# forbes110/taiwan-whisper

Hardware: AMD Instinct MI355X
Metric: distillation utterances/sec (30 s clips) (higher is better)
Workload: dtype bf16

## Files before the change

### include/tw_hip.h

```cpp
#ifndef TW_HIP_H
#define TW_HIP_H
#include <stdint.h>
#ifdef __cplusplus
extern "C" {
#endif

typedef void* tw_stream_t;

#define TW_GEMM_BIAS 1
#define TW_GEMM_ROUND 2
#define TW_GEMM_GELU 4
#define TW_GEMM_RES 8
#define TW_GEMM_ACCUM 16
#define TW_GEMM_AUX_OUT 32
#define TW_GEMM_DGELU 64
#define TW_GEMM_TILE128 256
#define TW_GEMM_TILE256 512
#define TW_GEMM_TILE256x128 1024
#define TW_GEMM_TILE256PP 2048
#define TW_GEMM_NOSPLIT 16384
#define TW_GEMM_TILE256x128_S2 262144
#define TW_GEMM_GROUP_M(g) ((g) << 24)


// ... 26 lines not shown
int tw_attn_fwd(const void* Q, int64_t ldq, const void* K, int64_t ldk, const void* V, int64_t ldv, void* O,
                int64_t ldo, float* lse, int B, int H, int Tq, int Tk, int head_dim, int causal, float scale,
                tw_stream_t stream);
int tw_attn_bwd(const void* Q, int64_t ldq, const void* K, int64_t ldk, const void* V, int64_t ldv, const void* O,
                int64_t ldo, const void* dO, int64_t lddo, const float* lse, void* dQ, int64_t lddq, void* dK,
                int64_t lddk, void* dV, int64_t lddv, int B, int H, int Tq, int Tk, int head_dim, int causal,
                float scale, float* workspace , tw_stream_t stream);
int tw_attn_fwd_varlen(const void* Q, int64_t ldq, const void* K, int64_t ldk, const void* V, int64_t ldv, void* O,
                       int64_t ldo, float* lse, const int* offq, const int* offk, int B, int H, int Mq, int max_q, int Tk,
                       int head_dim, int causal, float scale, tw_stream_t stream);
int tw_attn_fwd_varlen_f16(const void* Q, int64_t ldq, const void* K, int64_t ldk, const void* V, int64_t ldv, void* O,
                           int64_t ldo, float* lse, const int* offq, const int* offk, int B, int H, int Mq, int max_q,
                           int Tk, int head_dim, int causal, float scale, tw_stream_t stream);
int tw_attn_bwd_varlen(const void* Q, int64_t ldq, const void* K, int64_t ldk, const void* V, int64_t ldv,
                       const void* O, int64_t ldo, const void* dO, int64_t lddo, const float* lse, void* dQ,
                       int64_t lddq, void* dK, int64_t lddk, void* dV, int64_t lddv, const int* offq, const int* offk,
                       int B, int H, int Mq, int max_q, int Tk, int head_dim, int causal, float scale,
                       float* workspace , tw_stream_t stream);
int tw_attn_bwd_varlen_f16(const void* Q, int64_t ldq, const void* K, int64_t ldk, const void* V, int64_t ldv,
                           const void* O, int64_t ldo, const void* dO, int64_t lddo, const float* lse, void* dQ,
                           int64_t lddq, void* dK, int64_t lddk, void* dV, int64_t lddv, const int* offq,
                           const int* offk, int B, int H, int Mq, int max_q, int Tk, int head_dim, int causal,
                           float scale, float* workspace, tw_stream_t stream);

int tw_kl_ce(const void* s_logits, const void* t_logits, int64_t ld, int logits_dtype, const int64_t* labels,
             int64_t rows, int V, float T, float ce_w, float kl_w, const int* n_valid, float grad_scale, float* row_out,
             float* out3, void* dlogits, tw_stream_t stream);

int tw_logmel(const float* wav, int B, const float* basis, const int* mel_start, const float* mel_w, float* mel_out,
              void* conv_in, void* workspace , tw_stream_t stream);
int tw_logmel_len(const float* wav, int B, int64_t n_samples, const float* basis, const int* mel_start,
                  const float* mel_w, float* mel_out, void* conv_in, void* workspace, tw_stream_t stream);
int tw_logmel_mels(const float* wav, int B, int64_t n_samples, int n_mels, const float* basis, const int* mel_start,
                   const float* mel_w, float* mel_out, void* conv_in, void* workspace, tw_stream_t stream);
int tw_mel_to_conv_input(const float* mel, void* xt, int B, int nmel, int T, tw_stream_t stream);

int tw_embed_fwd(const int64_t* ids, const void* tok, int tok_dtype, const void* pos, int pos_dtype, void* out,
                 int out_dtype, int rows, int T, int pos_offset, int D, tw_stream_t stream);
int tw_embed_bwd(const int64_t* ids, const float* dh, float* dE, int rows, int D, int64_t padding_idx,
                 tw_stream_t stream);
int tw_pack_plan(const int64_t* labels, int B, int T, int* off, int64_t* src_rows, tw_stream_t stream);
int tw_embed_fwd_rows(const int64_t* ids, const int64_t* src_rows, const void* tok, int tok_dtype, const void* pos,
                      int pos_dtype, void* out, int out_dtype, int rows, int T, int pos_offset, int D,
                      tw_stream_t stream);
int tw_pos_grad_rows(const float* dx, const int* off, int B, int max_rows, int D, float* gP, tw_stream_t stream);

int tw_transpose_bf16(const void* src, int64_t ld_src, int rows, int cols, void* dst, int64_t ld_dst,
                      tw_stream_t stream);
int tw_cast_f32_bf16(const float* src, void* dst, int64_t n, tw_stream_t stream);
int tw_colsum(const void* x, int x_dtype, int64_t ldx, int rows, int cols, float* out, int accum, int round_bf16,
              float* workspace, int64_t workspace_floats, tw_stream_t stream);

int tw_l2norm(const float* x, int64_t n, float* norm_out, float* workspace , tw_stream_t stream);
int tw_adamw(float* p, const float* g, float* m, float* v, void* p_bf16, int64_t n, float lr, float b1, float b2,
             float eps, float wd, int step, const float* norm, float max_norm, tw_stream_t stream);
int tw_clip_scale(float* x, int64_t n, const float* norm, float max_norm, tw_stream_t stream);

int tw_im2col3(const void* src, int64_t src_rows, void* dst, int B, int T_out, int stride, int C,
               tw_stream_t stream);
int tw_col2im_s2(const float* dA, float* dX, int B, int T_in, int T_out, int C, tw_stream_t stream);
int tw_gelu_bwd(const void* g, int g_dtype, const void* pre, void* out, int64_t n, tw_stream_t stream);

int tw_shift_tokens_right(const int64_t* labels, int64_t* out, int B, int T, int64_t pad, int64_t start,
                          tw_stream_t stream);
// ... 116 lines not shown
```

### taiwan-whisper_amd/csrc/attention.hip

```cpp
#include "common.h"

#include <cstdlib>
#include <type_traits>

namespace {

constexpr int QW = 32;
constexpr int QB = 4 * QW;
constexpr int KT = 64;
constexpr int TB = KT * 64 * 2;

typedef __attribute__((address_space(3))) s16x4 lds_s16x4;

__device__ __forceinline__ int swz(int r, int c) { return r * 128 + ((c ^ (r & 7)) << 4); }

__device__ __forceinline__ void stage_tile(const bf16* base, int64_t ld, int rows_valid, char* lds, int wave,
                                           int lane) {
  const auto rs = make_rsrc(base);
#pragma unroll
  for (int i = 0; i < 2; ++i) {
    const int pce = wave + 4 * i;
    const int r = pce * 8 + (lane >> 3);
    const int c = (lane & 7) ^ (r & 7);
    const uint32_t off = r < rows_valid ? (uint32_t)(((int64_t)r * ld + c * 8) * 2) : TW_OOB;
// ... 32 lines not shown
}

template <bool H>
__device__ __forceinline__ void store4(bf16* dst, const f32x4& v) {
  *(bf16x4*)dst = bf16x4{f2e<H>(v[0]), f2e<H>(v[1]), f2e<H>(v[2]), f2e<H>(v[3])};
}

template <int N, int M>
__device__ __forceinline__ void zero(f32x4 (&a)[N][M]) {
#pragma unroll
  for (int i = 0; i < N; ++i)
#pragma unroll
    for (int j = 0; j < M; ++j) a[i][j] = f32x4{0.f, 0.f, 0.f, 0.f};
}

struct AttnP {
  const bf16* Q; const bf16* K; const bf16* V; bf16* O; float* lse;
  const bf16* dO; float* Dv; bf16* dQ; bf16* dK; bf16* dV;
  int64_t ldq, ldk, ldv, ldo, lddo, lddq, lddk, lddv;
  int B, H, Tq, Tk, causal;
  float scale, scale_log2;
  const int* offq; const int* offk;
  int Mq;
};

template <bool VL>
__device__ __forceinline__ void clip_rows(const int* off, int b, int& T, int64_t& row0) {
  row0 = (int64_t)b * T;
  if constexpr (VL) {
    if (off) {
      row0 = off[b];
      T = off[b + 1] - off[b];
    }
  }
}

constexpr float LOG2E = 1.4426950408889634f;

__device__ __forceinline__ void remap_bh(int& xblk, int& bh) {
  const int nx = gridDim.x, nwg = gridDim.x * gridDim.y;
  const int bid = blockIdx.y * nx + blockIdx.x;
  const int q = nwg / 8, rr = nwg % 8, xcd = bid % 8;
  const int tid = (xcd < rr ? xcd * (q + 1) : rr * (q + 1) + (xcd - rr) * q) + bid / 8;
  bh = tid / nx;
  xblk = tid % nx;
}
constexpr float NEG_BIG = -1e30f;

__device__ __forceinline__ float fmx(float a, float b) { return __builtin_elementwise_maximum(a, b); }

struct Frame {
  int lane, wave, g, li;
  int h;
  int blk, row;
  int Tq, Tk;
  int off;
  int64_t qrow0, krow0;
  int64_t lse0;
  const bf16 *Qb, *Kb, *Vb;
  template <class T> __device__ __forceinline__ T* qrow(T* base, int64_t ld, int r = 0) const {
    return base + (qrow0 + r) * ld + h * 64;
  }
  template <class T> __device__ __forceinline__ T* krow(T* base, int64_t ld, int r = 0) const {
    return base + (krow0 + r) * ld + h * 64;
  }
};

template <bool VL>
__device__ __forceinline__ Frame attn_frame(const AttnP& p) {
  Frame f;
  f.lane = lane_id();
  f.wave = wave_id_uniform();
  f.g = f.lane >> 4;
  f.li = f.lane & 15;
  int xblk, bh;
  remap_bh(xblk, bh);
  const int b = bh / p.H;
  f.h = bh % p.H;
  f.blk = xblk * QB;
  f.row = f.blk + f.wave * QW;
  f.Tq = p.Tq;
  f.Tk = p.Tk;
  clip_rows<VL>(p.offq, b, f.Tq, f.qrow0);
  clip_rows<VL>(p.offk, b, f.Tk, f.krow0);
  f.lse0 = VL ? (int64_t)f.h * p.Mq + f.qrow0 : (int64_t)bh * f.Tq;
  f.Qb = f.qrow(p.Q, p.ldq);
  f.Kb = f.krow(p.K, p.ldk);
  f.Vb = f.krow(p.V, p.ldv);
  f.off = f.Tk - f.Tq;
  return f;
}

__device__ __forceinline__ void stage_kv(const AttnP& p, const Frame& f, char* smem, int buf, int kt) {
  char* Ks = smem + buf * 2 * TB;
  const int k0 = kt * KT;
  stage_tile(f.Kb + (int64_t)k0 * p.ldk, p.ldk, f.Tk - k0, Ks, f.wave, f.lane);
  stage_tile(f.Vb + (int64_t)k0 * p.ldv, p.ldv, f.Tk - k0, Ks + TB, f.wave, f.lane);
}

__device__ __forceinline__ int causal_nkt(const AttnP& p, const Frame& f) {
  int nkt = (f.Tk + KT - 1) / KT;
  if (p.causal) {
// ... 374 lines not shown
    if (!(p.offq != nullptr && p.B > 0 && p.Mq >= 0 && p.Tq >= 0 && p.Tq <= p.Mq && p.Tk >= 0 &&
          !(p.causal && p.Tq > p.Tk)))
      return TW_EINVAL;
    if (p.Tk == 0 || (!bwd && (p.Mq == 0 || p.Tq == 0))) return TW_OK;
  } else if (p.B <= 0 || p.Tq <= 0 || p.Tk <= 0) {
    return TW_OK;
  }
  if ((((uintptr_t)p.Q | (uintptr_t)p.K | (uintptr_t)p.V) & 15) || ((p.ldq | p.ldk | p.ldv) & 7)) return TW_EINVAL;
  if (bwd ? (((uintptr_t)p.dO | (uintptr_t)p.O) & 15) || ((p.lddo | p.ldo) & 7) : (p.ldo & 3) != 0) return TW_EINVAL;
  if (!packed && p.causal && p.Tq > p.Tk) return TW_EINVAL;
  return ATTN_LAUNCH;
}

#define TW_DISPATCH_HVL(half, packed, ...)                                      \
  do {                                                                          \
    if ((half) && (packed)) { constexpr bool H = true, VL = true; __VA_ARGS__; } \
    else if (half) { constexpr bool H = true, VL = false; __VA_ARGS__; }        \
    else if (packed) { constexpr bool H = false, VL = true; __VA_ARGS__; }      \
    else { constexpr bool H = false, VL = false; __VA_ARGS__; }                 \
  } while (0)

dim3 attn_grid(const AttnP& p, int rows) { return dim3((rows + QB - 1) / QB, p.B * p.H); }

int attn_fwd(const AttnP& p, int head_dim, bool packed, bool half, hipStream_t stream) {
  if (const int st = attn_check(p, head_dim, packed, false); st != ATTN_LAUNCH) return st;
  TW_DISPATCH_HVL(half, packed,
                  hipLaunchKernelGGL((attn_fwd_kernel<H, VL>), attn_grid(p, p.Tq), dim3(256), 0, stream, p));
  TW_CHECK_LAUNCH();
  return TW_OK;
}

int attn_bwd(const AttnP& p, int head_dim, bool packed, bool half, hipStream_t stream) {
  if (const int st = attn_check(p, head_dim, packed, true); st != ATTN_LAUNCH) return st;
  TW_DISPATCH_HVL(half, packed, {
    if (p.Tq > 0)
      hipLaunchKernelGGL((attn_bwd_dq_kernel<H, VL>), attn_grid(p, p.Tq), dim3(256), 0, stream, p);
    hipLaunchKernelGGL((attn_bwd_dkdv_kernel<H, VL>), attn_grid(p, p.Tk), dim3(256), 0, stream, p);
  });
  TW_CHECK_LAUNCH();
  return TW_OK;
}

}

extern "C" int tw_attn_fwd(const void* Q, int64_t ldq, const void* K, int64_t ldk, const void* V, int64_t ldv, void* O,
                           int64_t ldo, float* lse, int B, int H, int Tq, int Tk, int head_dim, int causal, float scale,
                           hipStream_t stream) {
  return attn_fwd(attn_fill(Q, ldq, K, ldk, V, ldv, O, ldo, lse, B, H, Tq, Tk, causal, scale, nullptr, nullptr, 0),
                  head_dim, false, false, stream);
}

extern "C" int tw_attn_fwd_f16(const void* Q, int64_t ldq, const void* K, int64_t ldk, const void* V, int64_t ldv,
                               void* O, int64_t ldo, float* lse, int B, int H, int Tq, int Tk, int head_dim, int causal,
                               float scale, hipStream_t stream) {
  return attn_fwd(attn_fill(Q, ldq, K, ldk, V, ldv, O, ldo, lse, B, H, Tq, Tk, causal, scale, nullptr, nullptr, 0),
                  head_dim, false, true, stream);
}

extern "C" int tw_attn_bwd(const void* Q, int64_t ldq, const void* K, int64_t ldk, const void* V, int64_t ldv,
// ... 30 lines not shown
                  head_dim, true, true, stream);
}

extern "C" int tw_attn_bwd_varlen(const void* Q, int64_t ldq, const void* K, int64_t ldk, const void* V, int64_t ldv,
                                  const void* O, int64_t ldo, const void* dO, int64_t lddo, const float* lse, void* dQ,
                                  int64_t lddq, void* dK, int64_t lddk, void* dV, int64_t lddv, const int* offq,
                                  const int* offk, int B, int H, int Mq, int max_q, int Tk, int head_dim, int causal,
                                  float scale, float* workspace, hipStream_t stream) {
  return attn_bwd(attn_fill(Q, ldq, K, ldk, V, ldv, O, ldo, lse, B, H, max_q, Tk, causal, scale, offq, offk, Mq, dO,
                            lddo, dQ, lddq, dK, lddk, dV, lddv, workspace),
                  head_dim, true, false, stream);
}

extern "C" int tw_attn_bwd_varlen_f16(const void* Q, int64_t ldq, const void* K, int64_t ldk, const void* V,
                                      int64_t ldv, const void* O, int64_t ldo, const void* dO, int64_t lddo,
                                      const float* lse, void* dQ, int64_t lddq, void* dK, int64_t lddk, void* dV,
                                      int64_t lddv, const int* offq, const int* offk, int B, int H, int Mq, int max_q,
                                      int Tk, int head_dim, int causal, float scale, float* workspace,
                                      hipStream_t stream) {
  return attn_bwd(attn_fill(Q, ldq, K, ldk, V, ldv, O, ldo, lse, B, H, max_q, Tk, causal, scale, offq, offk, Mq, dO,
                            lddo, dQ, lddq, dK, lddk, dV, lddv, workspace),
                  head_dim, true, true, stream);
}
```

### taiwan-whisper_amd/csrc/misc.hip

```cpp
#include "common.h"

namespace {

__global__ void embed_fwd_kernel(const int64_t* __restrict__ ids, const void* __restrict__ tok, int tok_dtype,
                                 const void* __restrict__ pos, int pos_dtype, void* __restrict__ out, int out_dtype,
                                 int rows, int T, int pos_offset, int D) {
  const int row = blockIdx.x;
  if (row >= rows) return;
  const int64_t id = ids[row];
  const int t = row % T + pos_offset;
  for (int e = threadIdx.x; e < D; e += blockDim.x) {
    const float a = ld_as_f32(tok, tok_dtype, id * D + e);
    const float b = ld_as_f32(pos, pos_dtype, (int64_t)t * D + e);
    const float s = a + b;
    st_from_f32(out, out_dtype, (int64_t)row * D + e, s);
  }
}

__global__ __launch_bounds__(1024) void pack_plan_kernel(const int64_t* __restrict__ labels, int B, int T, int* off,
                                                         int64_t* __restrict__ src) {
  const int lane = threadIdx.x & 63, wv = threadIdx.x >> 6;
  for (int b = wv; b < B; b += 16) {
    int n = 0;
    for (int t = lane; t < T; t += 64)
      if (labels[(int64_t)b * T + t] >= 0) n = t + 1;
    for (int o = 32; o > 0; o >>= 1) n = max(n, __shfl_xor(n, o, 64));
    if (lane == 0) off[b + 1] = n;
  }
  __syncthreads();
  if (threadIdx.x == 0) {
    int s = 0;
    off[0] = 0;
    for (int b = 0; b < B; ++b) {
      s += off[b + 1];
      off[b + 1] = s;
    }
  }
  __syncthreads();
  for (int b = wv; b < B; b += 16) {
    const int r0 = off[b], n = off[b + 1] - r0;
    for (int t = lane; t < n; t += 64) src[r0 + t] = (int64_t)b * T + t;
  }
  for (int64_t i = off[B] + threadIdx.x; i < (int64_t)B * T; i += 1024) src[i] = 0;
}

__global__ void embed_fwd_rows_kernel(const int64_t* __restrict__ ids, const int64_t* __restrict__ src,
                                      const void* __restrict__ tok, int tok_dtype, const void* __restrict__ pos,
                                      int pos_dtype, void* __restrict__ out, int out_dtype, int rows, int T,
                                      int pos_offset, int D) {
  const int row = blockIdx.x;
  if (row >= rows) return;
  const int64_t id = ids[row];
  const int t = (int)(src[row] % T) + pos_offset;
  for (int e = threadIdx.x; e < D; e += blockDim.x) {
    const float a = ld_as_f32(tok, tok_dtype, id * D + e);
    const float b = ld_as_f32(pos, pos_dtype, (int64_t)t * D + e);
    st_from_f32(out, out_dtype, (int64_t)row * D + e, a + b);
  }
}

__global__ __launch_bounds__(256) void pos_grad_rows_kernel(const float* __restrict__ dx, const int* __restrict__ off,
                                                            int B, int D, float* __restrict__ gP) {
  const int t = blockIdx.x;
  const int e = blockIdx.y * 256 + threadIdx.x;
  if (e >= D) return;
  float acc = 0.f;
// ... 204 lines not shown
  if (b > cap) b = cap;
  if (b < 1) b = 1;
  return (int)b;
}

}

extern "C" int tw_embed_fwd(const int64_t* ids, const void* tok, int tok_dtype, const void* pos, int pos_dtype,
                            void* out, int out_dtype, int rows, int T, int pos_offset, int D, hipStream_t stream) {
  if (rows <= 0) return TW_OK;
  hipLaunchKernelGGL(embed_fwd_kernel, dim3(rows), dim3(256), 0, stream, ids, tok, tok_dtype, pos, pos_dtype, out,
                     out_dtype, rows, T, pos_offset, D);
  TW_CHECK_LAUNCH();
  return TW_OK;
}

extern "C" int tw_pack_plan(const int64_t* labels, int B, int T, int* off, int64_t* src_rows, hipStream_t stream) {
  if (B <= 0 || T <= 0) return TW_EINVAL;
  hipLaunchKernelGGL(pack_plan_kernel, dim3(1), dim3(1024), 0, stream, labels, B, T, off, src_rows);
  TW_CHECK_LAUNCH();
  return TW_OK;
}

extern "C" int tw_embed_fwd_rows(const int64_t* ids, const int64_t* src_rows, const void* tok, int tok_dtype,
                                 const void* pos, int pos_dtype, void* out, int out_dtype, int rows, int T,
                                 int pos_offset, int D, hipStream_t stream) {
  if (rows <= 0) return TW_OK;
  if (T <= 0) return TW_EINVAL;
  hipLaunchKernelGGL(embed_fwd_rows_kernel, dim3(rows), dim3(256), 0, stream, ids, src_rows, tok, tok_dtype, pos,
                     pos_dtype, out, out_dtype, rows, T, pos_offset, D);
  TW_CHECK_LAUNCH();
  return TW_OK;
}

extern "C" int tw_pos_grad_rows(const float* dx, const int* off, int B, int max_rows, int D, float* gP,
                                hipStream_t stream) {
  if (B <= 0 || max_rows <= 0 || D <= 0) return TW_OK;
  hipLaunchKernelGGL(pos_grad_rows_kernel, dim3(max_rows, (D + 255) / 256), dim3(256), 0, stream, dx, off, B, D, gP);
  TW_CHECK_LAUNCH();
  return TW_OK;
}

namespace {

__global__ __launch_bounds__(256) void transpose_bf16_kernel(const bf16* __restrict__ src, int64_t lds_, int rows,
                                                             int cols, bf16* __restrict__ dst, int64_t ldd, int vec) {
// ... 172 lines not shown
```

### taiwan-whisper_amd/tw/_native.py

```python
from __future__ import annotations

import ctypes
import os

_HERE = os.path.dirname(os.path.abspath(__file__))
LIB_PATH = os.environ.get("TW_HIP_LIB", os.path.join(_HERE, "_lib", "libtw_hip.so"))

P, I64, I32, F32 = ctypes.c_void_p, ctypes.c_int64, ctypes.c_int, ctypes.c_float

SIGNATURES = {
    "tw_gemm_bf16": [P, I64, I32, P, I64, I32, P, I64, I32, I32, I32, I32, I32, I64, I64, I64, F32, P,
                     P, I64, I64, I32, I32, P, I64, I64, I32, P],
    "tw_gemm_route": [P, I64, I32, P, I64, I32, P, I64, I32, I32, I32, I32, I32, I64, I64, I64, P,
                      P, I64, I64, I32, I32, P, I64, I64, I32, I32, I32, I32, P],
    "tw_flac_info": [P, I64, P],
    "tw_flac_decode": [P, I64, P, I64, P],
    "tw_gemv_bf16": [P, I64, P, P, F32, P, I64, P, I64, I32, I32, I32, I32, P, P, I64, I32, P, I64, I32,
                     P, I64, I64, I32, P, P],
    "tw_layernorm_fwd": [P, I32, P, P, P, I32, P, P, I32, I32, F32, P],
    "tw_layernorm_bwd": [P, I32, P, P, P, P, I32, P, I32, P, P, I32, I32, P, I64, P],
    "tw_layernorm_bwd_ex": [P, I32, P, P, P, P, I32, P, I32, P, P, I32, I32, P, I64, P, I32, P],
    "tw_add_layernorm_fwd": [P, I32, P, P, P, P, P, P, P, I32, I32, F32, P],
    "tw_attn_fwd": [P, I64, P, I64, P, I64, P, I64, P, I32, I32, I32, I32, I32, I32, F32, P],
    "tw_attn_bwd": [P, I64, P, I64, P, I64, P, I64, P, I64, P, P, I64, P, I64, P, I64, I32, I32, I32, I32,
                    I32, I32, F32, P, P],
    "tw_attn_fwd_varlen": [P, I64, P, I64, P, I64, P, I64, P, P, P, I32, I32, I32, I32, I32, I32, I32, F32, P],
    "tw_attn_fwd_varlen_f16": [P, I64, P, I64, P, I64, P, I64, P, P, P, I32, I32, I32, I32, I32, I32, I32, F32, P],
    "tw_attn_bwd_varlen": [P, I64, P, I64, P, I64, P, I64, P, I64, P, P, I64, P, I64, P, I64, P, P, I32, I32, I32,
                           I32, I32, I32, I32, F32, P, P],
    "tw_attn_bwd_varlen_f16": [P, I64, P, I64, P, I64, P, I64, P, I64, P, P, I64, P, I64, P, I64, P, P, I32, I32,
                               I32, I32, I32, I32, I32, F32, P, P],
    "tw_pack_plan": [P, I32, I32, P, P, P],
    "tw_embed_fwd_rows": [P, P, P, I32, P, I32, P, I32, I32, I32, I32, I32, P],
    "tw_pos_grad_rows": [P, P, I32, I32, I32, P, P],
    "tw_kl_ce": [P, P, I64, I32, P, I64, I32, F32, F32, F32, P, F32, P, P, P, P],
    "tw_logmel": [P, I32, P, P, P, P, P, P, P],
    "tw_logmel_len": [P, I32, I64, P, P, P, P, P, P, P],
    "tw_logmel_mels": [P, I32, I64, I32, P, P, P, P, P, P, P],
    "tw_mel_to_conv_input": [P, P, I32, I32, I32, P],
    "tw_embed_fwd": [P, P, I32, P, I32, P, I32, I32, I32, I32, I32, P],
    "tw_embed_bwd": [P, P, P, I32, I32, I64, P],
    "tw_cast_f32_bf16": [P, P, I64, P],
    "tw_transpose_bf16": [P, I64, I32, I32, P, I64, P],
    "tw_colsum": [P, I32, I64, I32, I32, P, I32, I32, P, I64, P],
    "tw_l2norm": [P, I64, P, P, P],
    "tw_adamw": [P, P, P, P, P, I64, F32, F32, F32, F32, F32, I32, P, F32, P],
    "tw_clip_scale": [P, I64, P, F32, P],
    "tw_im2col3": [P, I64, P, I32, I32, I32, I32, P],
    "tw_col2im_s2": [P, P, I32, I32, I32, I32, P],
    "tw_gelu_bwd": [P, I32, P, P, I64, P],
    "tw_shift_tokens_right": [P, P, I32, I32, I64, I64, P],
    "tw_count_valid": [P, I64, P, P],
    "tw_decode_attn": [P, I64, P, I64, I64, P, I64, I64, P, I64, I32, I32, I32, P, I32, F32, I32, P],
    "tw_decode_attn_hs": [P, I64, P, I64, I64, I64, P, I64, I64, I64, P, I64, I32, I32, I32, P, I32, F32, I32, P],
    "tw_decode_attn_ks": [P, I64, P, I64, I64, I64, P, I64, I64, I64, P, I64, I32, I32, I32, P, P, I32, F32, I32, P],
# ... 69 lines not shown
```

### taiwan-whisper_amd/tw/distill.py

```python
from __future__ import annotations

import contextlib
import math
import os
from typing import Optional

import torch

from . import ops as F
from .modeling import Backward, PackedRows, WhisperForConditionalGeneration, is_pseudo


def constant_with_warmup(step: int, warmup: int) -> float:
    if warmup > 0 and step < warmup:
        return step / warmup
    return 1.0


def linear_schedule(step: int, warmup: int, total: int) -> float:
    if warmup > 0 and step < warmup:
        return step / warmup
    return max(0.0, (total - step) / max(1, total - warmup))


# ... 126 lines not shown
        if self.sched == "constant":
            return self.lr
        return self.lr * constant_with_warmup(step, self.warmup)

    def _conv_input(self, batch):
        ci = batch.get("conv_input")
        if ci is not None and ci.dtype == self.s.act_dtype:
            return ci
        return self.s.conv_input(batch["input_features"])

    def _teacher_logits(self, conv_in, ids, labels, enc16, Tk, pk=None):
        t = self.t
        if self.share:
            t_ids = torch.empty_like(labels)
            F.shift_tokens_right(labels, t_ids, t.config.pad_token_id, t.config.decoder_start_token_id)
            ht = t.decode(t_ids if pk is None else pk.pack(t_ids), enc16, Tk, pk=pk)
        else:
            enc_t = t.encode(conv_in)
            ht = t.decode(ids if pk is None else pk.pack(ids), enc_t, Tk, pk=pk)
        return t.lm_head(ht)

    def _plan_rows(self, batch_labels, labels):
        B, T = labels.shape
        off = torch.empty(B + 1, dtype=torch.int32, device=labels.device)
        src = torch.empty(B * T, dtype=torch.int64, device=labels.device)
        F.pack_plan(labels, off, src)
        def descriptor(lens):
            pk = PackedRows(lens, off, src, T)
            return pk if pk.M > 0 else None

        if not batch_labels.is_cuda:
            pos = torch.arange(1, T + 1, dtype=torch.int64)
            lens = ((batch_labels >= 0) * pos).amax(1).tolist()
            return lambda: descriptor(lens)
        host = self._pin.get(B)
        if host is None:
            host = self._pin[B] = torch.empty(B + 1, dtype=torch.int32).pin_memory()
        host.copy_(off, non_blocking=True)
        ev = torch.cuda.Event()
        ev.record()

        def done():
            ev.synchronize()
            o = host.tolist()
            return descriptor([o[b + 1] - o[b] for b in range(B)])
        return done

    def train_step(self, batch, temperature: Optional[float] = None, end_of_dataloader: bool = False):
        T = self.temperature if temperature is None else temperature
        s = self.s
        conv_in = self._conv_input(batch)
        ids = batch["decoder_input_ids"].to(s.device).contiguous()
        labels = batch["labels"].to(s.device).contiguous()
        B, Td = ids.shape
        plan = self._plan_rows(batch["labels"], labels) if self.pack_rows else None
        enc_tape = [] if self.train_encoder else None
        enc16 = s.encode(conv_in, tape=enc_tape)
        self.flush()
        pk = plan() if plan is not None else None
        if self.micro == 0:
            s.grad.zero_()
        self._pending, self._reduced = [], []
        sync = self.micro + 1 == self.accum or end_of_dataloader
        self.bw.on_ready = self._grad_ready if (self.dp and sync) else None
        Tk = enc16.shape[0] // B
        tape = []
        with self._row_capacity(pk, B * Td):
            hs = s.decode(ids if pk is None else pk.pack(ids), enc16, Tk, tape=tape, pk=pk)
# ... 242 lines not shown
```

### taiwan-whisper_amd/tw/modeling.py

```python
from __future__ import annotations

import json
import math
import os
from dataclasses import dataclass
from typing import Optional

import numpy as np
import torch

from . import ops
from .config import GenerationConfig, WhisperConfig

_DEFER_RES = os.environ.get("TW_DEFER_RES", "1")
_LN_G16 = os.environ.get("TW_LN_G16", "1") != "0"

F = ops


def padded_vocab(V: int) -> int:
    return (V + 63) // 64 * 64



class PackedRows:

    def __init__(self, lens, off, src, T):
        self.lens = [int(n) for n in lens]
        self.B, self.T = len(self.lens), int(T)
        self.M, self.max_len = sum(self.lens), max(self.lens, default=0)
        if self.max_len > self.T or min(self.lens, default=0) < 0:
            raise ValueError("packed rows: a clip length outside [0, T]")
        if off.dtype != torch.int32 or off.numel() < self.B + 1 or src.dtype != torch.int64 or src.numel() < self.M:
            raise ValueError("packed rows: off is int32 [B+1], src int64 [>= M]")
        self.off, self.src = off, src[: self.M]

    @classmethod
    def from_lens(cls, lens, T, device):
        lens = [int(n) for n in lens]
        off = torch.tensor(np.concatenate([[0], np.cumsum(lens)]), dtype=torch.int32, device=device)
        src = torch.tensor([b * T + t for b, n in enumerate(lens) for t in range(n)], dtype=torch.int64, device=device)
        return cls(lens, off, src, T)

    def pack(self, x):
        if tuple(x.shape) != (self.B, self.T):
            raise ValueError(f"packed rows: expected [{self.B}, {self.T}], got {tuple(x.shape)}")
        return x.reshape(-1).index_select(0, self.src)


def fp32_compute_supported() -> bool:
    return True

def _attn_segs(p, d, fused_kv_only=False):
    segs = []
    if not fused_kv_only:
        segs += [(p + ".q_proj.weight", (d, d)), (p + ".k_proj.weight", (d, d)), (p + ".v_proj.weight", (d, d)),
                 (p + ".q_proj.bias", (d,)), (p + ".k_proj.zero_bias", (d,)), (p + ".v_proj.bias", (d,))]
    else:
# ... 420 lines not shown
        return xn, y

    def _res_out(self, h, w, b, x, tape, kind, clamp=False):
        M, N = h.shape[0], w.shape[0]
        if self.defer_residual(kind):
            r = self._rows(M, N, self.act_dtype)
            self._lin(h, w, b, r)
            return x, r
        out = self._rows(M, N, self.stream_dtype) if tape is not None else x
        flags = F.GEMM_ROUND | (F.GEMM_CLAMP16 if clamp and self.stream_dtype == torch.float16 else 0)
        self._lin(h, w, b, out, res=x, flags=flags)
        return out, None

    def _attn_fwd(self, x, p, q, ldq, k, v, ldkv, B, T, Tk, causal, tape, pk):
        d = self.config.d_model
        H = d // 64
        M = B * T if pk is None else pk.M
        o = self._rows(M, d, self.act_dtype)
        lse = torch.empty(H * M, dtype=torch.float32, device=self.device) if tape is not None else None
        if pk is None:
            F.attn_fwd(q, ldq, k, ldkv, v, ldkv, o, d, lse, B, H, T, T if Tk is None else Tk, causal, 0.125)
        else:
            offk, Tk = (pk.off, pk.max_len) if Tk is None else (None, Tk)
            F.attn_fwd_varlen(q, ldq, k, ldkv, v, ldkv, o, d, lse, pk.off, offk, pk.B, H, M, pk.max_len, Tk, causal, 0.125)
        out = self._res_out(o, self._w16(p + ".out_proj.weight"), self._w16(p + ".out_proj.bias"), x, tape, "attn")
        return out, o, lse

    def _attn_block(self, x, p, B, T, causal, tape=None, pend=None, pk=None):
        d = self.config.d_model
        sv = {} if tape is not None else None
        x, y = self._ln_in(x, pend, p + "_layer_norm", sv)
        M = B * T if pk is None else pk.M
        qkv = self._rows(M, 3 * d, self.act_dtype)
        wqkv = self.wspan(p + ".q_proj.weight", p + ".v_proj.weight", (3 * d, d))
        bqkv = self.wspan(p + ".q_proj.bias", p + ".v_proj.bias", (3 * d,))
        self._lin(y, wqkv, bqkv, qkv)
        out, o, lse = self._attn_fwd(x, p, qkv, 3 * d, qkv[:, d:], qkv[:, 2 * d:], 3 * d, B, T, None, causal, tape, pk)
        if tape is not None:
            tape.append(("attn", p, dict(sv=sv, y=y, qkv=qkv, o=o, lse=lse, B=B, T=T, causal=causal, pk=pk)))
        return out

    def _cross_block(self, x, enc16, p, B, T, Tk, tape=None, kv=None, pend=None, pk=None):
        d = self.config.d_model
        sv = {} if tape is not None else None
        x, y = self._ln_in(x, pend, p + "_layer_norm", sv)
        M = B * T if pk is None else pk.M
        q = self._rows(M, d, self.act_dtype)
# ... 260 lines not shown

    def _out_proj(self, p, st, dx):
        m = self.m
        d = m.config.d_model
        pk = st.get("pk")
        M = st["B"] * st["T"] if pk is None else pk.M
        g = self._grad16(dx)
        self.dW(g, st["o"], m.gv(p + ".out_proj.weight"), M)
        self.db(g, (0, d), m.gv(p + ".out_proj.bias"))
        do = m._rows(M, d, m.act_dtype)
        self.dX(g, m._w16(p + ".out_proj.weight"), do)
        return M, do

    def _attn_bwd(self, st, q, ldq, k, v, ldkv, do, dq, lddq, dk, dv, lddkv, Tk, causal):
        d = self.m.config.d_model
        H = d // 64
        B, T, pk = st["B"], st["T"], st.get("pk")
        if pk is None:
            F.attn_bwd(q, ldq, k, ldkv, v, ldkv, st["o"], d, do, d, st["lse"], dq, lddq, dk, lddkv, dv, lddkv, B, H, T,
                       T if Tk is None else Tk, causal, 0.125)
        else:
            offk, Tk = (pk.off, pk.max_len) if Tk is None else (None, Tk)
            F.attn_bwd_varlen(q, ldq, k, ldkv, v, ldkv, st["o"], d, do, d, st["lse"], dq, lddq, dk, lddkv, dv, lddkv,
                              pk.off, offk, pk.B, H, pk.M, pk.max_len, Tk, causal, 0.125)

    def attn(self, p, st, dx):
        m = self.m
        d = m.config.d_model
        M, do = self._out_proj(p, st, dx)
        qkv = st["qkv"]
        dqkv = m._rows(M, 3 * d, m.act_dtype)
        self._attn_bwd(st, qkv, 3 * d, qkv[:, d:], qkv[:, 2 * d:], 3 * d, do, dqkv, 3 * d, dqkv[:, d:], dqkv[:, 2 * d:],
                       3 * d, None, st["causal"])
        self.dW(dqkv, st["y"], self.span_grad(p + ".q_proj.weight", p + ".v_proj.weight", (3 * d, d)), M)
        self.db(dqkv, (0, d), m.gv(p + ".q_proj.bias"))
        self.db(dqkv, (2 * d, 3 * d), m.gv(p + ".v_proj.bias"))
        dy = m._rows(M, d, m.act_dtype)
        wqkv = m.wspan(p + ".q_proj.weight", p + ".v_proj.weight", (3 * d, d))
        self.dX(dqkv, wqkv, dy)
        self.ln(st["sv"], p + "_layer_norm", dy, dx)

    def cross(self, p, st, dx, enc16, d_enc):
        m = self.m
        d = m.config.d_model
        B, Tk = st["B"], st["Tk"]
        M, do = self._out_proj(p, st, dx)
        kv = st["kv"]
# ... 119 lines not shown
```

### taiwan-whisper_amd/tw/ops.py

```python
from __future__ import annotations

import collections
import ctypes

import torch

from ._native import call
from .profiling import KernelTimer

F32, BF16, F16 = 0, 1, 2
GEMM_BIAS, GEMM_ROUND, GEMM_GELU, GEMM_RES, GEMM_ACCUM, GEMM_AUX_OUT, GEMM_DGELU = 1, 2, 4, 8, 16, 32, 64
GEMM_CLAMP16 = 128
HALF = (torch.bfloat16, torch.float16)
GEMM_TILE128, GEMM_TILE256, GEMM_TILE256x128, GEMM_TILE256PP = 256, 512, 1024, 2048
GEMM_NOSPLIT = 16384
GEMM_TILE256x128_S2 = 262144


def GEMM_GROUP_M(g: int) -> int:
    assert 0 < g < 16
    return g << 24


GEMM_ROUTES = ("skinny", "skinny_splitk", "splitk_dw", "rounds_sk_tail", "rounds_dp_tail", "persistent",
# ... 197 lines not shown
def attn_fwd(q, ldq, k, ldk, v, ldv, o, ldo, lse, B, H, Tq, Tk, causal, scale):
    if q.dtype == torch.float32:
        return attn_fwd_f32(q, ldq, k, ldk, v, ldv, o, ldo, lse, B, H, Tq, Tk, causal, scale)
    sym = _attn_sym("attn_fwd", q, ((q, ldq, "q"), (o, ldo, "o")), ((k, ldk, "k"), (v, ldv, "v")), lse, H, B, Tq, Tk)
    call(sym, q.data_ptr(), ldq, k.data_ptr(), ldk, v.data_ptr(), ldv, o.data_ptr(), ldo, _ptr(lse), B, H, Tq, Tk, 64,
         int(causal), float(scale), _stream())
    return o


def attn_bwd(q, ldq, k, ldk, v, ldv, o, ldo, do, lddo, lse, dq, lddq, dk, lddk, dv, lddv, B, H, Tq, Tk, causal,
             scale, workspace=None):
    if q.dtype == torch.float32:
        return attn_bwd_f32(q, ldq, k, ldk, v, ldv, o, ldo, do, lddo, lse, dq, lddq, dk, lddk, dv, lddv, B, H, Tq, Tk,
                            causal, scale)
    sym = _attn_sym("attn_bwd", q, ((q, ldq, "q"), (o, ldo, "o"), (do, lddo, "do"), (dq, lddq, "dq")),
                    ((k, ldk, "k"), (v, ldv, "v"), (dk, lddk, "dk"), (dv, lddv, "dv")), lse, H, B, Tq, Tk)
    if workspace is None or workspace.numel() < B * H * Tq:
        workspace = torch.empty(B * H * Tq, dtype=torch.float32, device=q.device)
    call(sym, q.data_ptr(), ldq, k.data_ptr(), ldk, v.data_ptr(), ldv, o.data_ptr(), ldo, do.data_ptr(), lddo,
         lse.data_ptr(), dq.data_ptr(), lddq, dk.data_ptr(), lddk, dv.data_ptr(), lddv, B, H, Tq, Tk, 64, int(causal),
         float(scale), workspace.data_ptr(), _stream())


def attn_fwd_varlen(q, ldq, k, ldk, v, ldv, o, ldo, lse, offq, offk, B, H, Mq, max_q, Tk, causal, scale):
    sym = _attn_sym("attn_fwd_varlen", q, ((q, ldq, "q"), (o, ldo, "o")), ((k, ldk, "k"), (v, ldv, "v")), lse, H, B,
                    max_q, Tk, offq, offk, Mq)
    if sym is not None:
        call(sym, q.data_ptr(), ldq, k.data_ptr(), ldk, v.data_ptr(), ldv, o.data_ptr(), ldo, _ptr(lse),
             offq.data_ptr(), _ptr(offk), B, H, Mq, max_q, Tk, 64, int(causal), float(scale), _stream())
    return o


def attn_bwd_varlen(q, ldq, k, ldk, v, ldv, o, ldo, do, lddo, lse, dq, lddq, dk, lddk, dv, lddv, offq, offk, B, H, Mq,
                    max_q, Tk, causal, scale):
    sym = _attn_sym("attn_bwd_varlen", q, ((q, ldq, "q"), (o, ldo, "o"), (do, lddo, "do"), (dq, lddq, "dq")),
                    ((k, ldk, "k"), (v, ldv, "v"), (dk, lddk, "dk"), (dv, lddv, "dv")), lse, H, B, max_q, Tk, offq,
                    offk, Mq)
    if sym is None:
        return
    ws = torch.empty(max(H * Mq, 1), dtype=torch.float32, device=q.device)
    call(sym, q.data_ptr(), ldq, k.data_ptr(), ldk, v.data_ptr(), ldv, o.data_ptr(), ldo, do.data_ptr(), lddo,
         lse.data_ptr(), dq.data_ptr(), lddq, dk.data_ptr(), lddk, dv.data_ptr(), lddv, offq.data_ptr(), _ptr(offk), B,
         H, Mq, max_q, Tk, 64, int(causal), float(scale), ws.data_ptr(), _stream())


def kl_ce(s_logits, t_logits, labels, V, n_valid, T=2.0, ce_w=0.8, kl_w=1.0, grad_scale=1.0, dlogits=None,
          row_out=None, out3=None):
    rows, ld = s_logits.shape
    assert t_logits.shape == s_logits.shape and s_logits.dtype == t_logits.dtype
    assert s_logits.dtype in (torch.bfloat16, torch.float16, torch.float32)
    assert labels.dtype == torch.int64 and labels.numel() == rows and n_valid.dtype == torch.int32
    if row_out is None:
        row_out = torch.empty(rows * 2, dtype=torch.float32, device=s_logits.device)
    if out3 is None:
        out3 = torch.empty(3, dtype=torch.float32, device=s_logits.device)
    if dlogits is not None:
        assert dlogits.shape == s_logits.shape and dlogits.dtype == s_logits.dtype
        assert dlogits.data_ptr() != t_logits.data_ptr(), "kl_ce: dlogits may alias the student logits, not the teacher's"
    call("tw_kl_ce", s_logits.data_ptr(), t_logits.data_ptr(), ld, _dt(s_logits), labels.data_ptr(), rows, V, float(T),
         float(ce_w), float(kl_w), n_valid.data_ptr(), float(grad_scale), row_out.data_ptr(), out3.data_ptr(),
         _ptr(dlogits), _stream())
    return out3, row_out


def logmel(wav, basis, mel_start, mel_w, mel_out, conv_in=None, workspace=None):
    B, n = wav.shape
# ... 27 lines not shown
        return xt
    assert xt.dtype in HALF
    call("tw_mel_to_conv_input_f16" if xt.dtype == torch.float16 else "tw_mel_to_conv_input", mel.data_ptr(),
         xt.data_ptr(), B, nmel, T, _stream())
    return xt


def embed_fwd(ids, tok, pos, out, T, pos_offset=0):
    rows = ids.numel()
    D = tok.shape[1]
    assert ids.dtype == torch.int64 and out.shape[-1] == D and out.numel() == rows * D
    assert pos.shape[0] >= T + pos_offset
    call("tw_embed_fwd", ids.data_ptr(), tok.data_ptr(), _dt(tok), pos.data_ptr(), _dt(pos), out.data_ptr(),
         _dt(out), rows, T, pos_offset, D, _stream())
    return out


def pack_plan(labels, off, src_rows):
    B, T = labels.shape
    assert labels.dtype == torch.int64 and labels.is_contiguous() and labels.is_cuda
    assert off.dtype == torch.int32 and src_rows.dtype == torch.int64
    _need(off, B + 1, "pack_plan off"); _need(src_rows, B * T, "pack_plan src_rows")
    call("tw_pack_plan", labels.data_ptr(), B, T, off.data_ptr(), src_rows.data_ptr(), _stream())


def embed_fwd_rows(ids, src_rows, tok, pos, out, T, pos_offset=0):
    rows = ids.numel()
    D = tok.shape[1]
    assert ids.dtype == torch.int64 and src_rows.dtype == torch.int64 and ids.is_contiguous()
    assert out.shape[-1] == D and out.numel() == rows * D and out.is_contiguous()
    assert pos.shape[0] >= T + pos_offset
    _need(src_rows, rows, "embed src_rows")
    call("tw_embed_fwd_rows", ids.data_ptr(), src_rows.data_ptr(), tok.data_ptr(), _dt(tok), pos.data_ptr(), _dt(pos),
         out.data_ptr(), _dt(out), rows, T, pos_offset, D, _stream())
    return out


def pos_grad_rows(dx, off, B, M, max_rows, gP):
    D = gP.shape[1]
    assert dx.dtype == torch.float32 and gP.dtype == torch.float32 and off.dtype == torch.int32
    assert gP.is_contiguous() and gP.shape[0] >= max_rows and 0 <= max_rows <= M
    _need(off, B + 1, "pos_grad off")
    if M > 0:
        _need(dx, M * D, "pos_grad dx")
    call("tw_pos_grad_rows", dx.data_ptr(), off.data_ptr(), B, max_rows, D, gP.data_ptr(), _stream())

# ... 496 lines not shown
```

Measured before the change: 269.7.

## Launch varlen attention over a compact list of live query blocks

Adds a GPU kernel that builds a compact list of (batch, query-block) entries for packed variable-length decoder sequences. For causal attention the list is sorted by KV tile count, longest first. The varlen attention forward and dQ backward kernels are then launched over this list instead of a max_q-by-B grid, so workgroups that would find no valid rows are never created and heavy blocks start first. It adds a small single-workgroup O(n^2) ranking kernel per step and a custom block-to-head placement, and it depends on block counts matching the host-side lengths.

```diff
diff --git a/include/tw_hip.h b/include/tw_hip.h
--- a/include/tw_hip.h
+++ b/include/tw_hip.h
@@ -72,6 +72,24 @@
                            int64_t lddq, void* dK, int64_t lddk, void* dV, int64_t lddv, const int* offq,
                            const int* offk, int B, int H, int Mq, int max_q, int Tk, int head_dim, int causal,
                            float scale, float* workspace, tw_stream_t stream);
+int tw_attn_fwd_blocks(const void* Q, int64_t ldq, const void* K, int64_t ldk, const void* V, int64_t ldv, void* O,
+                       int64_t ldo, float* lse, const int* offq, const int* offk, const int* blocks, int nblk,
+                       int B, int H, int Mq, int max_q, int Tk, int head_dim, int causal, float scale,
+                       tw_stream_t stream);
+int tw_attn_fwd_blocks_f16(const void* Q, int64_t ldq, const void* K, int64_t ldk, const void* V, int64_t ldv, void* O,
+                           int64_t ldo, float* lse, const int* offq, const int* offk, const int* blocks, int nblk,
+                           int B, int H, int Mq, int max_q, int Tk, int head_dim, int causal, float scale,
+                           tw_stream_t stream);
+int tw_attn_bwd_blocks(const void* Q, int64_t ldq, const void* K, int64_t ldk, const void* V, int64_t ldv,
+                       const void* O, int64_t ldo, const void* dO, int64_t lddo, const float* lse, void* dQ,
+                       int64_t lddq, void* dK, int64_t lddk, void* dV, int64_t lddv, const int* offq, const int* offk,
+                       const int* blocks, int nblk, int B, int H, int Mq, int max_q, int Tk, int head_dim, int causal,
+                       float scale, float* workspace , tw_stream_t stream);
+int tw_attn_bwd_blocks_f16(const void* Q, int64_t ldq, const void* K, int64_t ldk, const void* V, int64_t ldv,
+                           const void* O, int64_t ldo, const void* dO, int64_t lddo, const float* lse, void* dQ,
+                           int64_t lddq, void* dK, int64_t lddk, void* dV, int64_t lddv, const int* offq,
+                           const int* offk, const int* blocks, int nblk, int B, int H, int Mq, int max_q, int Tk,
+                           int head_dim, int causal, float scale, float* workspace, tw_stream_t stream);
 
 int tw_kl_ce(const void* s_logits, const void* t_logits, int64_t ld, int logits_dtype, const int64_t* labels,
              int64_t rows, int V, float T, float ce_w, float kl_w, const int* n_valid, float grad_scale, float* row_out,
@@ -90,6 +108,7 @@
 int tw_embed_bwd(const int64_t* ids, const float* dh, float* dE, int rows, int D, int64_t padding_idx,
                  tw_stream_t stream);
 int tw_pack_plan(const int64_t* labels, int B, int T, int* off, int64_t* src_rows, tw_stream_t stream);
+int tw_pack_blocks(const int* off, int B, int max_rows, int* blocks, int cap, int* nblk, tw_stream_t stream);
 int tw_embed_fwd_rows(const int64_t* ids, const int64_t* src_rows, const void* tok, int tok_dtype, const void* pos,
                       int pos_dtype, void* out, int out_dtype, int rows, int T, int pos_offset, int D,
                       tw_stream_t stream);
diff --git a/taiwan-whisper_amd/csrc/attention.hip b/taiwan-whisper_amd/csrc/attention.hip
--- a/taiwan-whisper_amd/csrc/attention.hip
+++ b/taiwan-whisper_amd/csrc/attention.hip
@@ -78,6 +78,7 @@
   float scale, scale_log2;
   const int* offq; const int* offk;
   int Mq;
+  const int4* wl;
 };
 
 template <bool VL>
@@ -122,6 +123,25 @@
   }
 };
 
+__device__ __forceinline__ void place_entry(bool causal, int& ent, int& h) {
+  if (!causal) {
+    remap_bh(h, ent);
+    return;
+  }
+  const int H = gridDim.x, nent = gridDim.y;
+  const int bid = blockIdx.y * H + blockIdx.x;
+  const int full = nent & ~7;
+  if (bid < full * H) {
+    const int t = bid >> 3;
+    h = t % H;
+    ent = (t / H) * 8 + (bid & 7);
+  } else {
+    const int local = bid - full * H, r = nent - full;
+    ent = full + local % r;
+    h = local / r;
+  }
+}
+
 template <bool VL>
 __device__ __forceinline__ Frame attn_frame(const AttnP& p) {
   Frame f;
@@ -129,11 +149,20 @@
   f.wave = wave_id_uniform();
   f.g = f.lane >> 4;
   f.li = f.lane & 15;
-  int xblk, bh;
-  remap_bh(xblk, bh);
-  const int b = bh / p.H;
-  f.h = bh % p.H;
-  f.blk = xblk * QB;
+  int b, bh = 0;
+  if (VL && p.wl) {
+    int ent;
+    place_entry(p.causal, ent, f.h);
+    const int4 e = p.wl[ent];
+    b = e.x;
+    f.blk = e.y;
+  } else {
+    int xblk;
+    remap_bh(xblk, bh);
+    b = bh / p.H;
+    f.h = bh % p.H;
+    f.blk = xblk * QB;
+  }
   f.row = f.blk + f.wave * QW;
   f.Tq = p.Tq;
   f.Tk = p.Tk;
@@ -554,19 +583,44 @@
 
 dim3 attn_grid(const AttnP& p, int rows) { return dim3((rows + QB - 1) / QB, p.B * p.H); }
 
-int attn_fwd(const AttnP& p, int head_dim, bool packed, bool half, hipStream_t stream) {
+struct Blocks {
+  const int* list;
+  int n;
+};
+
+dim3 list_grid(const AttnP& p, const Blocks& bl) { return dim3(p.H, bl.n); }
+AttnP with_list(AttnP p, const Blocks& bl) {
+  p.wl = (const int4*)bl.list;
+  return p;
+}
+
+int blocks_check(const Blocks& bl) {
+  return bl.list != nullptr && ((uintptr_t)bl.list & 15) == 0 && bl.n >= 0 && bl.n <= 65535 ? TW_OK : TW_EINVAL;
+}
+
+int attn_fwd(const AttnP& p, int head_dim, bool packed, bool half, hipStream_t stream, const Blocks* bl = nullptr) {
   if (const int st = attn_check(p, head_dim, packed, false); st != ATTN_LAUNCH) return st;
+  if (bl) {
+    if (const int st = blocks_check(*bl); st != TW_OK) return st;
+    if (bl->n == 0) return TW_OK;
+  }
+  const AttnP pl = bl ? with_list(p, *bl) : p;
   TW_DISPATCH_HVL(half, packed,
-                  hipLaunchKernelGGL((attn_fwd_kernel<H, VL>), attn_grid(p, p.Tq), dim3(256), 0, stream, p));
+                  hipLaunchKernelGGL((attn_fwd_kernel<H, VL>), bl ? list_grid(p, *bl) : attn_grid(p, p.Tq), dim3(256), 0,
+                                     stream, pl));
   TW_CHECK_LAUNCH();
   return TW_OK;
 }
 
-int attn_bwd(const AttnP& p, int head_dim, bool packed, bool half, hipStream_t stream) {
+int attn_bwd(const AttnP& p, int head_dim, bool packed, bool half, hipStream_t stream, const Blocks* bl = nullptr) {
   if (const int st = attn_check(p, head_dim, packed, true); st != ATTN_LAUNCH) return st;
+  if (bl)
+    if (const int st = blocks_check(*bl); st != TW_OK) return st;
+  const AttnP pq = bl ? with_list(p, *bl) : p;
   TW_DISPATCH_HVL(half, packed, {
-    if (p.Tq > 0)
-      hipLaunchKernelGGL((attn_bwd_dq_kernel<H, VL>), attn_grid(p, p.Tq), dim3(256), 0, stream, p);
+    if (bl ? bl->n > 0 : p.Tq > 0)
+      hipLaunchKernelGGL((attn_bwd_dq_kernel<H, VL>), bl ? list_grid(p, *bl) : attn_grid(p, p.Tq), dim3(256), 0,
+                         stream, pq);
     hipLaunchKernelGGL((attn_bwd_dkdv_kernel<H, VL>), attn_grid(p, p.Tk), dim3(256), 0, stream, p);
   });
   TW_CHECK_LAUNCH();
@@ -643,3 +697,44 @@
                             lddo, dQ, lddq, dK, lddk, dV, lddv, workspace),
                   head_dim, true, true, stream);
 }
+
+extern "C" int tw_attn_fwd_blocks(const void* Q, int64_t ldq, const void* K, int64_t ldk, const void* V, int64_t ldv,
+                                  void* O, int64_t ldo, float* lse, const int* offq, const int* offk,
+                                  const int* blocks, int nblk, int B, int H, int Mq, int max_q, int Tk, int head_dim,
+                                  int causal, float scale, hipStream_t stream) {
+  const Blocks bl = {blocks, nblk};
+  return attn_fwd(attn_fill(Q, ldq, K, ldk, V, ldv, O, ldo, lse, B, H, max_q, Tk, causal, scale, offq, offk, Mq),
+                  head_dim, true, false, stream, &bl);
+}
+
+extern "C" int tw_attn_fwd_blocks_f16(const void* Q, int64_t ldq, const void* K, int64_t ldk, const void* V,
+                                      int64_t ldv, void* O, int64_t ldo, float* lse, const int* offq, const int* offk,
+                                      const int* blocks, int nblk, int B, int H, int Mq, int max_q, int Tk,
+                                      int head_dim, int causal, float scale, hipStream_t stream) {
+  const Blocks bl = {blocks, nblk};
+  return attn_fwd(attn_fill(Q, ldq, K, ldk, V, ldv, O, ldo, lse, B, H, max_q, Tk, causal, scale, offq, offk, Mq),
+                  head_dim, true, true, stream, &bl);
+}
+
+extern "C" int tw_attn_bwd_blocks(const void* Q, int64_t ldq, const void* K, int64_t ldk, const void* V, int64_t ldv,
+                                  const void* O, int64_t ldo, const void* dO, int64_t lddo, const float* lse, void* dQ,
+                                  int64_t lddq, void* dK, int64_t lddk, void* dV, int64_t lddv, const int* offq,
+                                  const int* offk, const int* blocks, int nblk, int B, int H, int Mq, int max_q, int Tk,
+                                  int head_dim, int causal, float scale, float* workspace, hipStream_t stream) {
+  const Blocks bl = {blocks, nblk};
+  return attn_bwd(attn_fill(Q, ldq, K, ldk, V, ldv, O, ldo, lse, B, H, max_q, Tk, causal, scale, offq, offk, Mq, dO,
+                            lddo, dQ, lddq, dK, lddk, dV, lddv, workspace),
+                  head_dim, true, false, stream, &bl);
+}
+
+extern "C" int tw_attn_bwd_blocks_f16(const void* Q, int64_t ldq, const void* K, int64_t ldk, const void* V,
+                                      int64_t ldv, const void* O, int64_t ldo, const void* dO, int64_t lddo,
+                                      const float* lse, void* dQ, int64_t lddq, void* dK, int64_t lddk, void* dV,
+                                      int64_t lddv, const int* offq, const int* offk, const int* blocks, int nblk,
+                                      int B, int H, int Mq, int max_q, int Tk, int head_dim, int causal,
+                                      float scale, float* workspace, hipStream_t stream) {
+  const Blocks bl = {blocks, nblk};
+  return attn_bwd(attn_fill(Q, ldq, K, ldk, V, ldv, O, ldo, lse, B, H, max_q, Tk, causal, scale, offq, offk, Mq, dO,
+                            lddo, dQ, lddq, dK, lddk, dV, lddv, workspace),
+                  head_dim, true, true, stream, &bl);
+}
diff --git a/taiwan-whisper_amd/csrc/misc.hip b/taiwan-whisper_amd/csrc/misc.hip
--- a/taiwan-whisper_amd/csrc/misc.hip
+++ b/taiwan-whisper_amd/csrc/misc.hip
@@ -42,6 +42,37 @@
     for (int t = lane; t < n; t += 64) src[r0 + t] = (int64_t)b * T + t;
   }
   for (int64_t i = off[B] + threadIdx.x; i < (int64_t)B * T; i += 1024) src[i] = 0;
+}
+
+__global__ __launch_bounds__(1024) void pack_blocks_kernel(const int* __restrict__ off, int B, int max_rows,
+                                                           int4* __restrict__ blocks, int cap, int* nblk) {
+  const int mb = (max_rows + 127) / 128;
+  auto key = [&](int list, int b, int k, int n) -> uint64_t {
+    const int tiles = list ? (min(n, k * 128 + 128) + 63) / 64 : 0;
+    return ((uint64_t)(0xfffff - tiles) << 40) | ((uint64_t)b << 16) | (uint64_t)k;
+  };
+  for (int c = threadIdx.x; c < B * mb; c += 1024) {
+    const int b = c / mb, k = c % mb;
+    const int n = min(off[b + 1] - off[b], max_rows);
+    if (k * 128 >= n) continue;
+    const uint64_t k0 = key(0, b, k, n), k1 = key(1, b, k, n);
+    int r0 = 0, r1 = 0;
+    for (int b2 = 0; b2 < B; ++b2) {
+      const int n2 = min(off[b2 + 1] - off[b2], max_rows);
+      for (int k2 = 0; k2 * 128 < n2; ++k2) {
+        r0 += key(0, b2, k2, n2) < k0;
+        r1 += key(1, b2, k2, n2) < k1;
+      }
+    }
+    const int rows = min(128, n - k * 128);
+    if (r0 < cap) blocks[r0] = int4{b, k * 128, rows, 0};
+    if (r1 < cap) blocks[cap + r1] = int4{b, k * 128, rows, (min(n, k * 128 + 128) + 63) / 64};
+  }
+  if (threadIdx.x == 0) {
+    int nb = 0;
+    for (int b = 0; b < B; ++b) nb += (max(min(off[b + 1] - off[b], max_rows), 0) + 127) / 128;
+    *nblk = nb;
+  }
 }
 
 __global__ void embed_fwd_rows_kernel(const int64_t* __restrict__ ids, const int64_t* __restrict__ src,
@@ -292,6 +323,16 @@
   return TW_OK;
 }
 
+extern "C" int tw_pack_blocks(const int* off, int B, int max_rows, int* blocks, int cap, int* nblk,
+                              hipStream_t stream) {
+  if (B <= 0 || max_rows < 0 || !off || !blocks || !nblk || ((uintptr_t)blocks & 15) ||
+      (int64_t)cap < (int64_t)B * ((max_rows + 127) / 128))
+    return TW_EINVAL;
+  hipLaunchKernelGGL(pack_blocks_kernel, dim3(1), dim3(1024), 0, stream, off, B, max_rows, (int4*)blocks, cap, nblk);
+  TW_CHECK_LAUNCH();
+  return TW_OK;
+}
+
 extern "C" int tw_embed_fwd_rows(const int64_t* ids, const int64_t* src_rows, const void* tok, int tok_dtype,
                                  const void* pos, int pos_dtype, void* out, int out_dtype, int rows, int T,
                                  int pos_offset, int D, hipStream_t stream) {
diff --git a/taiwan-whisper_amd/tw/_native.py b/taiwan-whisper_amd/tw/_native.py
--- a/taiwan-whisper_amd/tw/_native.py
+++ b/taiwan-whisper_amd/tw/_native.py
@@ -30,7 +30,15 @@
                            I32, I32, I32, I32, F32, P, P],
     "tw_attn_bwd_varlen_f16": [P, I64, P, I64, P, I64, P, I64, P, I64, P, P, I64, P, I64, P, I64, P, P, I32, I32,
                                I32, I32, I32, I32, I32, F32, P, P],
+    "tw_attn_fwd_blocks": [P, I64, P, I64, P, I64, P, I64, P, P, P, P, I32, I32, I32, I32, I32, I32, I32, I32, F32, P],
+    "tw_attn_fwd_blocks_f16": [P, I64, P, I64, P, I64, P, I64, P, P, P, P, I32, I32, I32, I32, I32, I32, I32, I32, F32,
+                               P],
+    "tw_attn_bwd_blocks": [P, I64, P, I64, P, I64, P, I64, P, I64, P, P, I64, P, I64, P, I64, P, P, P, I32, I32, I32,
+                           I32, I32, I32, I32, I32, F32, P, P],
+    "tw_attn_bwd_blocks_f16": [P, I64, P, I64, P, I64, P, I64, P, I64, P, P, I64, P, I64, P, I64, P, P, P, I32, I32,
+                               I32, I32, I32, I32, I32, I32, F32, P, P],
     "tw_pack_plan": [P, I32, I32, P, P, P],
+    "tw_pack_blocks": [P, I32, I32, P, I32, P, P],
     "tw_embed_fwd_rows": [P, P, P, I32, P, I32, P, I32, I32, I32, I32, I32, P],
     "tw_pos_grad_rows": [P, P, I32, I32, I32, P, P],
     "tw_kl_ce": [P, P, I64, I32, P, I64, I32, F32, F32, F32, P, F32, P, P, P, P],
diff --git a/taiwan-whisper_amd/tw/distill.py b/taiwan-whisper_amd/tw/distill.py
--- a/taiwan-whisper_amd/tw/distill.py
+++ b/taiwan-whisper_amd/tw/distill.py
@@ -172,11 +172,14 @@
 
     def _plan_rows(self, batch_labels, labels):
         B, T = labels.shape
-        off = torch.empty(B + 1, dtype=torch.int32, device=labels.device)
+        plan = torch.empty(B + 2, dtype=torch.int32, device=labels.device)
+        off, nblk = plan[: B + 1], plan[B + 1:]
         src = torch.empty(B * T, dtype=torch.int64, device=labels.device)
+        blocks = PackedRows.new_blocks(B, T, labels.device)
         F.pack_plan(labels, off, src)
-        def descriptor(lens):
-            pk = PackedRows(lens, off, src, T)
+        F.pack_blocks(off, B, T, blocks, nblk)
+        def descriptor(lens, nblk=None):
+            pk = PackedRows(lens, off, src, T, blocks, nblk)
             return pk if pk.M > 0 else None
 
         if not batch_labels.is_cuda:
@@ -185,15 +188,15 @@
             return lambda: descriptor(lens)
         host = self._pin.get(B)
         if host is None:
-            host = self._pin[B] = torch.empty(B + 1, dtype=torch.int32).pin_memory()
-        host.copy_(off, non_blocking=True)
+            host = self._pin[B] = torch.empty(B + 2, dtype=torch.int32).pin_memory()
+        host.copy_(plan, non_blocking=True)
         ev = torch.cuda.Event()
         ev.record()
 
         def done():
             ev.synchronize()
             o = host.tolist()
-            return descriptor([o[b + 1] - o[b] for b in range(B)])
+            return descriptor([o[b + 1] - o[b] for b in range(B)], o[B + 1])
         return done
 
     def train_step(self, batch, temperature: Optional[float] = None, end_of_dataloader: bool = False):
diff --git a/taiwan-whisper_amd/tw/modeling.py b/taiwan-whisper_amd/tw/modeling.py
--- a/taiwan-whisper_amd/tw/modeling.py
+++ b/taiwan-whisper_amd/tw/modeling.py
@@ -25,7 +25,7 @@
 
 class PackedRows:
 
-    def __init__(self, lens, off, src, T):
+    def __init__(self, lens, off, src, T, blocks=None, nblk=None):
         self.lens = [int(n) for n in lens]
         self.B, self.T = len(self.lens), int(T)
         self.M, self.max_len = sum(self.lens), max(self.lens, default=0)
@@ -34,6 +34,20 @@
         if off.dtype != torch.int32 or off.numel() < self.B + 1 or src.dtype != torch.int64 or src.numel() < self.M:
             raise ValueError("packed rows: off is int32 [B+1], src int64 [>= M]")
         self.off, self.src = off, src[: self.M]
+        want = sum((n + 127) // 128 for n in self.lens)
+        if blocks is None and self.M > 0:
+            blocks = self.new_blocks(self.B, self.T, off.device)
+            F.pack_blocks(off, self.B, self.T, blocks, torch.empty(1, dtype=torch.int32, device=off.device))
+        if nblk is not None and int(nblk) != want:
+            raise ValueError(f"packed rows: {nblk} blocks do not match the lengths ({want})")
+        self.blocks, self.nblk = blocks, want
+
+    @staticmethod
+    def new_blocks(B, T, device):
+        return torch.empty(2, max(B * ((T + 127) // 128), 1), 4, dtype=torch.int32, device=device)
+
+    def block_list(self, causal):
+        return self.blocks[1 if causal else 0], self.nblk
 
     @classmethod
     def from_lens(cls, lens, T, device):
@@ -500,7 +514,8 @@
             F.attn_fwd(q, ldq, k, ldkv, v, ldkv, o, d, lse, B, H, T, T if Tk is None else Tk, causal, 0.125)
         else:
             offk, Tk = (pk.off, pk.max_len) if Tk is None else (None, Tk)
-            F.attn_fwd_varlen(q, ldq, k, ldkv, v, ldkv, o, d, lse, pk.off, offk, pk.B, H, M, pk.max_len, Tk, causal, 0.125)
+            F.attn_fwd_varlen(q, ldq, k, ldkv, v, ldkv, o, d, lse, pk.off, offk, pk.B, H, M, pk.max_len, Tk, causal, 0.125,
+                              blocks=pk.block_list(causal))
         out = self._res_out(o, self._w16(p + ".out_proj.weight"), self._w16(p + ".out_proj.bias"), x, tape, "attn")
         return out, o, lse
 
@@ -807,7 +822,8 @@
         else:
             offk, Tk = (pk.off, pk.max_len) if Tk is None else (None, Tk)
             F.attn_bwd_varlen(q, ldq, k, ldkv, v, ldkv, st["o"], d, do, d, st["lse"], dq, lddq, dk, lddkv, dv, lddkv,
-                              pk.off, offk, pk.B, H, pk.M, pk.max_len, Tk, causal, 0.125)
+                              pk.off, offk, pk.B, H, pk.M, pk.max_len, Tk, causal, 0.125,
+                              blocks=pk.block_list(causal))
 
     def attn(self, p, st, dx):
         m = self.m
diff --git a/taiwan-whisper_amd/tw/ops.py b/taiwan-whisper_amd/tw/ops.py
--- a/taiwan-whisper_amd/tw/ops.py
+++ b/taiwan-whisper_amd/tw/ops.py
@@ -243,26 +243,38 @@
          float(scale), workspace.data_ptr(), _stream())
 
 
-def attn_fwd_varlen(q, ldq, k, ldk, v, ldv, o, ldo, lse, offq, offk, B, H, Mq, max_q, Tk, causal, scale):
+def _block_args(sym, blocks):
+    if blocks is None:
+        return sym, ()
+    wl, nblk = blocks
+    assert wl.dtype == torch.int32 and wl.is_contiguous() and wl.numel() >= 4 * nblk
+    return sym.replace("_varlen", "_blocks"), (wl.data_ptr(), int(nblk))
+
+
+def attn_fwd_varlen(q, ldq, k, ldk, v, ldv, o, ldo, lse, offq, offk, B, H, Mq, max_q, Tk, causal, scale, blocks=None):
     sym = _attn_sym("attn_fwd_varlen", q, ((q, ldq, "q"), (o, ldo, "o")), ((k, ldk, "k"), (v, ldv, "v")), lse, H, B,
                     max_q, Tk, offq, offk, Mq)
     if sym is not None:
+        sym, bl = _block_args(sym, blocks)
         call(sym, q.data_ptr(), ldq, k.data_ptr(), ldk, v.data_ptr(), ldv, o.data_ptr(), ldo, _ptr(lse),
-             offq.data_ptr(), _ptr(offk), B, H, Mq, max_q, Tk, 64, int(causal), float(scale), _stream())
+             offq.data_ptr(), _ptr(offk), *bl, B, H, Mq, max_q, Tk, 64, int(causal), float(scale), _stream())
     return o
 
 
 def attn_bwd_varlen(q, ldq, k, ldk, v, ldv, o, ldo, do, lddo, lse, dq, lddq, dk, lddk, dv, lddv, offq, offk, B, H, Mq,
-                    max_q, Tk, causal, scale):
+                    max_q, Tk, causal, scale, blocks=None, workspace=None):
     sym = _attn_sym("attn_bwd_varlen", q, ((q, ldq, "q"), (o, ldo, "o"), (do, lddo, "do"), (dq, lddq, "dq")),
                     ((k, ldk, "k"), (v, ldv, "v"), (dk, lddk, "dk"), (dv, lddv, "dv")), lse, H, B, max_q, Tk, offq,
                     offk, Mq)
     if sym is None:
         return
-    ws = torch.empty(max(H * Mq, 1), dtype=torch.float32, device=q.device)
+    sym, bl = _block_args(sym, blocks)
+    ws = workspace
+    if ws is None or ws.numel() < H * Mq:
+        ws = torch.empty(max(H * Mq, 1), dtype=torch.float32, device=q.device)
     call(sym, q.data_ptr(), ldq, k.data_ptr(), ldk, v.data_ptr(), ldv, o.data_ptr(), ldo, do.data_ptr(), lddo,
-         lse.data_ptr(), dq.data_ptr(), lddq, dk.data_ptr(), lddk, dv.data_ptr(), lddv, offq.data_ptr(), _ptr(offk), B,
-         H, Mq, max_q, Tk, 64, int(causal), float(scale), ws.data_ptr(), _stream())
+         lse.data_ptr(), dq.data_ptr(), lddq, dk.data_ptr(), lddk, dv.data_ptr(), lddv, offq.data_ptr(), _ptr(offk),
+         *bl, B, H, Mq, max_q, Tk, 64, int(causal), float(scale), ws.data_ptr(), _stream())
 
 
 def kl_ce(s_logits, t_logits, labels, V, n_valid, T=2.0, ce_w=0.8, kl_w=1.0, grad_scale=1.0, dlogits=None,
@@ -336,6 +348,14 @@
     assert off.dtype == torch.int32 and src_rows.dtype == torch.int64
     _need(off, B + 1, "pack_plan off"); _need(src_rows, B * T, "pack_plan src_rows")
     call("tw_pack_plan", labels.data_ptr(), B, T, off.data_ptr(), src_rows.data_ptr(), _stream())
+
+
+def pack_blocks(off, B, max_rows, blocks, nblk):
+    assert off.dtype == torch.int32 and blocks.dtype == torch.int32 and nblk.dtype == torch.int32
+    assert blocks.dim() == 3 and blocks.shape[0] == 2 and blocks.shape[2] == 4 and blocks.is_contiguous()
+    _need(off, B + 1, "pack_blocks off"); _need(nblk, 1, "pack_blocks nblk")
+    call("tw_pack_blocks", off.data_ptr(), B, int(max_rows), blocks.data_ptr(), blocks.shape[1], nblk.data_ptr(),
+         _stream())
 
 
 def embed_fwd_rows(ids, src_rows, tok, pos, out, T, pos_offset=0):
```

Measured after the change: 274.8, median of 6. +1.9%, better.
